# matthewT53/JPEG-Encoder-and-Decoder

Hardware: AMD Instinct MI355X
Metric: Mpixels/sec RGB→quantised-coeff, 4K 4:4:4 q=90; % HBM roofline (higher is better)
Workload: dtype f32; 1 GPU; 8 x 3840x2160 RGB frames per GPU, 4:4:4, q=90, block-row stripes; global_batch_frames=8, width=3840, height=2160, quality=90, parallelism=stripes1, collectives=none, kernel_timing=HIP events around the K launches on their stream, launch=eager, input_sets=2

## Files before the change

jpeg-encoder-and-decoder_amd/csrc/jpgx_internal.h:

```cpp
#ifndef JPGX_INTERNAL_H
#define JPGX_INTERNAL_H

#include <stddef.h>
#include <stdint.h>

#include "../../include/jpgx.h"

#define JX_WG 256

struct jx_udiv {
    uint32_t m, s1, s2;
};
static inline struct jx_udiv jx_udiv_make(uint32_t d)
{
    unsigned l = 0;
    while (l < 32 && (1ull << l) < (unsigned long long)d) l++;
    struct jx_udiv r;
    r.m = (uint32_t)(((1ull << 32) * ((1ull << l) - d)) / d + 1);
    r.s1 = l ? 1u : 0u;
    r.s2 = l ? l - 1u : 0u;
    return r;
}

struct jx_geom {
    const uint8_t *rgb;
    int16_t *out;
    long long in_pitch;
    long long in_fstride;
    long long out_fstride;
    int bpr;
    int nb;
    int nframes;
    int row0;
    uint32_t under[6];
    struct jx_udiv dnb, dbpr;
    uint32_t mpr, nmcu;
    struct jx_udiv dmpr, dnmcu;
};

struct jx_qtab {
    float w[3][8][8];
    int16_t q[2][64];
};

struct jx_limtab {
    float lim[3][8][8];
};

#define JX_MAXQ 97

#ifndef JX_MX_PARTS
#define JX_MX_PARTS 2
#endif
#ifndef JX_MX_LOEXP
#define JX_MX_LOEXP 0
#endif
struct jx_mxtab {
    float w[24][8];
    float lsq[24][8];
    int16_t q[2][64];
    double r[2][64];
};

struct jx_xform_args {
    struct jx_geom g;
    int quality;
    int force_exact;
    int luma_only;
    int sub;
};


#ifdef __cplusplus
extern "C" {
#endif
int jx_plan_tables(int quality, float w[3][64], float lim[3][64], int16_t q[2][64]);
int jx_plan_tables_mode(int quality, int sub, float w[3][64], float lim[3][64], int16_t q[2][64]);
void jx_under_dwords(const uint8_t under[3][8], uint32_t out[6]);
long long jx_selftest_pk(long long nblocks, unsigned long long seed);
int jx_mx_parts(void);
int jx_mx_loexp(void);
int jx_plan_tables_mx(int quality, float w[24][8], float lim[24][8], int16_t q[2][64]);
int jx_plan_tables_mx422(int quality, float w[24][8], float lim[24][8], int16_t q[2][64]);
int jx_plan_tables_mx420(int quality, float w[24][8], float lim[24][8], int16_t q[2][64]);
int jx_mx_operands(uint16_t ops[3 * JX_MX_PARTS][64][8]);
int jx_mx422_operands(uint16_t ops[JX_MX_PARTS][4][64][8]);
int jx_mx420_operands(uint16_t ops[JX_MX_PARTS][5][64][8]);
long long jx_selftest_mx(long long nblocks, unsigned long long seed, int quality,
                         long long *flagged, double *ratio);
long long jx_selftest_mx422(long long nblocks, unsigned long long seed, int quality,
                            long long *flagged, double *ratio);
long long jx_selftest_mx420(long long nblocks, unsigned long long seed, int quality,
                            long long *flagged, double *ratio);
int jx_launch_mx(const struct jx_xform_args *xa, int sr, void *stream, void *ev_start, void *ev_stop);
long long jx_mx_image(int sr, int force, int quality, void *dst, long long cap);
int jx_launch_alt(const struct jx_xform_args *xa, int sr, size_t nbc, void *stream, void *ev_start, void *ev_stop);
#define JX_JFIF_HDR_MAX 768
void jx_jfif_build_codes(const uint8_t bits[16], const uint8_t *vals, uint32_t cl[256]);
void jx_jfif_codes(uint32_t cl[4][256]);
size_t jx_jfif_header(int width, int height, int quality, int sample_ratio, unsigned ri,
                      uint8_t *out, size_t cap);
#define JX_JFIF_DHT_STD 432
size_t jx_jfif_header_tabs(int width, int height, int quality, int sample_ratio, unsigned ri,
                           const uint8_t bits[4][16], const uint8_t vals[4][256], uint8_t *out,
                           size_t cap, size_t *dht_at);
int jx_jfif_optimal(const uint64_t counts[256], uint8_t bits[16], uint8_t vals[256]);
#ifdef __cplusplus
}
#endif

#endif
```

jpeg-encoder-and-decoder_amd/csrc/jpgx_mx.hip:

```cpp
#include <hip/hip_ext.h>
#include <hip/hip_runtime.h>
#include <math.h>
#include <stdint.h>
#include <string.h>

#include <algorithm>
#include <memory>
#include <mutex>
#include <type_traits>
#include <vector>

#include "jpgx_internal.h"
#include "jx_consts.h"
#include "jx_hip.h"
#include "xform_math.h"

#pragma clang fp contract(off)

namespace {

typedef _Float16 mx_h8 __attribute__((ext_vector_type(8)));
typedef _Float16 mx_h2 __attribute__((ext_vector_type(2)));
typedef float mx_f4 __attribute__((ext_vector_type(4)));
typedef uint32_t mx_u4 __attribute__((ext_vector_type(4)));
// ... 339 lines not shown
        if (__popc(b1) == 1 && one(sl, (unsigned)__builtin_ctz(b1))) bits = 0;
    }
}

__device__ __forceinline__ bool mx_put_one(const void *stage, unsigned off, bool ok, int val)
{
    if (!__builtin_amdgcn_readfirstlane((int)ok)) return false;
    if (mx_lane() == 0) *(__attribute__((address_space(3))) int16_t *)(mx_lds((void *)stage) + off) = (int16_t)val;
    return true;
}

__device__ __forceinline__ unsigned mx_col_block(unsigned k, unsigned sl)
{
    const unsigned gg = sl >> 4, jj = sl & 15u;
    return k == 0 ? gg : (k == 1 ? 4u + gg : (jj < 8 ? gg : 4u + gg));
}

template <class Lds, class XT>
__device__ __forceinline__ void mx_exact_inline(Lds &L, const uint8_t *slot, uint32_t bits,
                                                const XT &xt)
{
    const unsigned lane = mx_lane();
    mx_wave_sync();
    mx_exact_single(bits, [&](unsigned sl, unsigned bt) __attribute__((always_inline)) {
        const unsigned k = bt >> 3, v = bt & 7u;
        const unsigned jj = sl & 15u, u = jj & 7u, ch = k < 2 ? (jj >> 3) : 2u;
        const unsigned jb = mx_col_block(k, sl);
        int val;
        const bool ok = mx_exact_one(MxSmp1{mx_lds((void *)slot) + 24u * jb, 192u}, ch, u, v, xt, val);
        return mx_put_one(L.stage, mxs_coef(mx_pos(ch, jb), xt.scan(u, v)), ok, val);
    });
    for (;;) {
        const uint64_t act = __ballot(bits != 0);
        if (!act) break;
        const int rk = mx_rank(act);
        if (bits != 0 && rk < 8) {
            const unsigned b = (unsigned)__builtin_ctz(bits);
            bits &= bits - 1u;
            L.task[rk] = (uint16_t)(lane << 8 | b);
        }
        mx_wave_sync();
        const int nt = std::min((int)__popcll(act), 8);
        const unsigned i = lane >> 3, x = lane & 7u;
        const bool live = (int)i < nt;
        const unsigned code = L.task[live ? i : 0u];
        const unsigned sl = code >> 8, k = (code >> 3) & 3u, v = code & 7u;
        const unsigned jj = sl & 15u, u = jj & 7u, ch = k < 2 ? (jj >> 3) : 2u;
        const unsigned jb = mx_col_block(k, sl);
        const int val = mx_exact_coef<true>(MxSmp1{mx_lds((void *)slot) + 24u * jb, 192u}, ch, u, v, x, xt);
        if (live && x == 7)
            *(__attribute__((address_space(3))) int16_t *)(mx_lds(L.stage) + mxs_coef(mx_pos(ch, jb), xt.scan(u, v))) =
                (int16_t)val;
        mx_wave_sync();
    }
}

__device__ __forceinline__ void mx_unpack8(const mx_f4 &a, const mx_f4 &b, float (&o)[8])
{
    o[0] = a.x, o[4] = a.y, o[2] = a.z, o[6] = a.w;
    o[1] = b.x, o[3] = b.y, o[5] = b.z, o[7] = b.w;
}

__device__ __forceinline__ uint32_t mx_flags(const float (&F)[8], const float (&W)[8], const float (&Lq)[8])
{
    uint32_t m = 0;
#pragma unroll
    for (int k = 0; k < 8; k++) {
        const float tm = __builtin_fmaf(F[k], W[k], kMagic);
        const float rr = tm - kMagic;
        const float d = __builtin_fmaf(F[k], W[k], -rr);
        const float e = __builtin_fmaf(d, d, -Lq[k]);
        m |= (e >= 0.0f ? 1u : 0u) << k;
    }
    return m;
}

static_assert(JX_MX_LOEXP == 0, "the kernels take R = acc_h + acc_l");
__device__ __forceinline__ void mx_combine(mx_f4 hl, mx_f4 ll, mx_f4 hh, mx_f4 lh, float (&R)[8])
{
    R[0] = ll.x + hl.x, R[1] = ll.y + hl.y, R[2] = ll.z + hl.z, R[3] = ll.w + hl.w;
    R[4] = lh.x + hh.x, R[5] = lh.y + hh.y, R[6] = lh.z + hh.z, R[7] = lh.w + hh.w;
}

struct MxW {
    mx_f4 w01, w23;
};
__device__ __forceinline__ MxW mx_w(const MxTab &tb, unsigned t0, unsigned j)
{
    return MxW{tb.wl[t0][0][j], tb.wl[t0][1][j]};
}
__device__ __forceinline__ MxW mx_l(const MxTab &tb, unsigned t0, unsigned j)
{
    return MxW{tb.wl[t0 + 1][0][j], tb.wl[t0 + 1][1][j]};
}
struct MxsTab {
    mx_f4 yc[2][2][16];
    mx_f4 cr[2][2][8];
};
__device__ __forceinline__ MxW mx_w(const MxsTab &tb, unsigned t0, unsigned j)
{
    return t0 == 0 ? MxW{tb.yc[0][0][j], tb.yc[0][1][j]} : MxW{tb.cr[0][0][j & 7u], tb.cr[0][1][j & 7u]};
}
__device__ __forceinline__ MxW mx_l(const MxsTab &tb, unsigned t0, unsigned j)
{
    return t0 == 0 ? MxW{tb.yc[1][0][j], tb.yc[1][1][j]} : MxW{tb.cr[1][0][j & 7u], tb.cr[1][1][j & 7u]};
}
__host__ __device__ __forceinline__ float mx_limc(const MxTab &tb, unsigned t, unsigned j)
{
    const mx_f4 a = tb.wl[t][0][j], b = tb.wl[t][1][j];
    const float mn = fminf(fminf(fminf(a.x, a.y), fminf(a.z, a.w)), fminf(fminf(b.x, b.y), fminf(b.z, b.w)));
    if (!(mn >= 0.0f)) return -1.0f;
    return (float)sqrt((double)mn) * (1.0f - 0x1p-20f);
}

__device__ __forceinline__ void mx_fence(const mx_f4 &r)
{
    const uint32_t v = __builtin_amdgcn_readfirstlane(__float_as_uint(r.w));
    asm volatile("" ::"s"(v) : "memory");
}

template <int N>
__device__ __forceinline__ void mx_fence_all(const mx_f4 (&r)[N])
{
    uint32_t v = 0;
#pragma unroll
    for (int i = 0; i < N; i++) v += __float_as_uint(r[i].w);
    asm volatile("" ::"v"(v) : "memory");
}

__device__ __forceinline__ void mx_keep(const mx_f4 (&x)[4])
{
    asm volatile("" ::"v"(x[0]), "v"(x[1]), "v"(x[2]), "v"(x[3]));
}
template <class T>
__device__ __forceinline__ int mx_keep1(const T &x)
{
    asm volatile("" ::"v"(x));
    return 0;
}
template <class... T>
__device__ __forceinline__ void mx_keep_ops(const T &...x)
{
    const int k[] = {mx_keep1(x)...};
    (void)k;
}

template <unsigned OFF, class TB>
__device__ __forceinline__ void mx_column_r(const float (&R)[8], const MxW &t, float limc, const TB &tb,
                                             unsigned t0, unsigned j, const uint32_t (&za)[8], uint32_t &fl, int kc,
                                             const mx_f4 *fence = nullptr)
{
    float F[8], W[8];
    jx_fdct8<FOps>(R, F);
    mx_unpack8(t.w01, t.w23, W);
    typedef __attribute__((address_space(3))) uint16_t l16;
    float em = 0.0f;
#pragma unroll
    for (int p = 0; p < 4; p++) {
        const int k0 = jx_pk_k(p, 0), k1 = jx_pk_k(p, 1);
        const float t0v = __builtin_fmaf(F[k0], W[k0], kMagic), t1v = __builtin_fmaf(F[k1], W[k1], kMagic);
        *(l16 *)(uintptr_t)(za[k0] + OFF) = (uint16_t)__float_as_uint(t0v);
        *(l16 *)(uintptr_t)(za[k1] + OFF) = (uint16_t)__float_as_uint(t1v);
        const float d0 = __builtin_fmaf(F[k0], W[k0], -(t0v - kMagic));
        const float d1 = __builtin_fmaf(F[k1], W[k1], -(t1v - kMagic));
        em = __builtin_fmaxf(__builtin_fmaxf(em, __builtin_fabsf(d0)), __builtin_fabsf(d1));
    }
    if (__builtin_expect(__ballot(em >= limc) != 0, 0)) {
        if (fence) mx_fence(*fence);
        const MxW lw = mx_l(tb, t0, j);
        float Lq[8];
        mx_unpack8(lw.w01, lw.w23, Lq);
        fl |= mx_flags(F, W, Lq) << (8 * kc);
    }
}

struct MxNoKeep {
    __device__ void operator()() const {}
};
template <unsigned OFF, bool LAZY = false, class TB, class KF = MxNoKeep>
__device__ __forceinline__ void mx_column_t(const mx_f4 (&acc)[4], const MxW &t, float limc, const TB &tb,
                                             unsigned t0, unsigned j, const uint32_t (&za)[8], uint32_t &fl, int kc,
                                             const mx_f4 *fence = nullptr, const KF &keep = KF{})
{
    float R[8];
    mx_combine(acc[0], acc[1], acc[2], acc[3], R);
    if (LAZY) {
        __builtin_amdgcn_sched_barrier(0);
        if (fence) mx_fence(*fence);
        keep();
        mx_column_r<OFF>(R, mx_w(tb, t0, j), limc, tb, t0, j, za, fl, kc, nullptr);
    } else {
        keep();
        mx_column_r<OFF>(R, t, limc, tb, t0, j, za, fl, kc, fence);
    }
}

constexpr unsigned kMxsC = 3;
constexpr unsigned kMxsWPG = 4;
struct alignas(16) MxsLds {
    uint8_t ring[kMxsC][kSlot];
    uint8_t stage[24 * kBSs];
    uint16_t task[8];
};
static_assert(sizeof(MxsLds) % 16 == 0, "16-byte aligned LDS regions");
__device__ mx_u4 g_mxs_B[3 * JX_MX_PARTS][64];
struct alignas(16) MxsImg {
    MxsTab tab;
    float limc[2][16];
    uint8_t scan_t[8][8];
    MxExTab ex;
};
constexpr unsigned kMxsPieces = sizeof(MxsImg) / 16;
static_assert(sizeof(MxsImg) % 16 == 0 && kMxsPieces <= 768, "three 16-byte pieces per thread");
static_assert(sizeof(MxsLds) * kMxsWPG + sizeof(MxsImg) <= 40 * 1024, "4 workgroups of 4 waves per CU");
__device__ MxsImg g_mxs_img[2][JX_MAXQ + 1];

template <unsigned N>
__device__ __forceinline__ void mx_wait_vm()
{
    static_assert(N < 64, "vmcnt is 6 bits");
    __builtin_amdgcn_s_waitcnt((int)((N & 15u) | ((N >> 4) << 14) | 0xF70u));
}

template <int SIZE>
__device__ __forceinline__ void mxs_dma(const void *g, void *lds)
{
    static_assert(SIZE == 16 || SIZE == 4, "dwordx4 or dword pieces");
    if constexpr (SIZE == 16)
        __builtin_amdgcn_global_load_lds((mx_gp)g, (mx_lp)lds, 16, 0, 0);
    else
        __builtin_amdgcn_global_load_lds((mx_gp)g, (mx_lp)lds, 4, 0, 0);
}

struct MxsCur {
    unsigned b, c;
    bool simple;
    const uint8_t *src;
    int16_t *dst;
    int16_t *cdst;
};

__device__ __forceinline__ void mxs_simple(MxsCur &P, const MxG &g)
{
    P.simple = P.c + 8u < g.bpr && P.b + 8u <= g.total && g.lin_store;
}

__device__ __forceinline__ void mxs_at(MxsCur &P, const MxG &g, unsigned b)
{
    P.b = b;
    P.simple = false;
    if (b >= g.total) return;
    MxCur X;
    mx_seek(X, g, b);
    P.c = X.c;
    P.src = X.src;
    P.dst = X.dst;
    P.cdst = g.out + (long long)X.f * g.ofstride + 64ll * (g.nb + X.bi / 2u);
    mxs_simple(P, g);
}

__device__ __forceinline__ void mxs_next(MxsCur &P, const MxG &g)
{
    if (!P.simple) {
        mxs_at(P, g, P.b + 8u);
        return;
    }
    P.b += 8u;
    P.c += 8u;
    P.src += 192;
    P.dst += 512;
    P.cdst += 256;
    mxs_simple(P, g);
}

__device__ __forceinline__ void mxs_issue(const MxsCur &P, const MxG &g, uint8_t *slot, uint32_t off0,
                                          uint32_t off1, unsigned lane)
{
    if (P.simple) {
        mxs_dma<16>(P.src + off0, slot);
        if (lane < 32) mxs_dma<16>(P.src + off1, slot + 1024u);
    } else {
        mxs_dma<4>(g.rgb, slot);
        mxs_dma<4>(g.rgb, slot);
    }
}

__global__ __launch_bounds__(64 * kMxsWPG, kWPE) void k_mxs(const jx_xform_args a)
{
    __shared__ __attribute__((aligned(16))) MxsLds s_lds[kMxsWPG];
    __shared__ __attribute__((aligned(16))) MxsImg s_img;
    MxG g;
    g.rgb = a.g.rgb;
    g.out = a.g.out;
    g.pitch = a.g.in_pitch;
    g.fstride = a.g.in_fstride;
    g.ofstride = a.g.out_fstride;
    g.bpr = (unsigned)a.g.bpr;
    g.nb = (unsigned)a.g.nb;
    g.total = (unsigned)a.g.nb * (unsigned)a.g.nframes;
    g.row0 = a.g.row0;
    g.quality = a.quality;
    g.force = a.force_exact;
    g.lin_store = (unsigned long long)g.nb * 256ull + 1024ull < (1ull << 31);
#pragma unroll
    for (int k = 0; k < 6; k++) g.u[k] = a.g.under[k];
    g.dnb = a.g.dnb;
    g.dbpr = a.g.dbpr;

    const unsigned lane = threadIdx.x & 63u;
    const unsigned wave = __builtin_amdgcn_readfirstlane(threadIdx.x >> 6);
    MxsLds &L = s_lds[wave];
    mx_u4 B[kParts][3];
#pragma unroll
    for (int p = 0; p < kParts; p++)
#pragma unroll
        for (int w = 0; w < 3; w++) B[p][w] = g_mxs_B[3 * p + w][lane];
    {
        const uint8_t *img = (const uint8_t *)&g_mxs_img[g.force ? 1 : 0][g.quality];
#pragma unroll
        for (unsigned i = 0; i < (kMxsPieces + 64u * kMxsWPG - 1u) / (64u * kMxsWPG); i++) {
            const unsigned piece = 64u * kMxsWPG * i + threadIdx.x;
            if (64u * kMxsWPG * i + 64u * wave < kMxsPieces && piece < kMxsPieces)
                mxs_dma<16>(img + 16u * piece, (uint8_t *)&s_img + 16u * (64u * kMxsWPG * i + 64u * wave));
        }
    }
    const unsigned wv = blockIdx.x * kMxsWPG + wave;
    const uint32_t off0 = (uint32_t)((lane / 12u) * (unsigned)g.pitch + 16u * (lane % 12u));
    const uint32_t off1 = (uint32_t)(((64u + lane) / 12u) * (unsigned)g.pitch + 16u * ((64u + lane) % 12u));
    MxsCur iss;
    mxs_at(iss, g, 8u * kMxsC * wv);
    MxsCur cmp = iss;
#pragma unroll
    for (unsigned k = 0; k < kMxsC; k++) {
        mxs_issue(iss, g, L.ring[k], off0, off1, lane);
        mxs_next(iss, g);
    }

    const unsigned m = lane & 15u, q = lane >> 4;
    const uint32_t aoff = 192u * (m & 3u) + 24u * (m >> 2) + 8u * (q < 3 ? q : 2u);
    const uint32_t s0 = q < 3 ? kSelLo : kSelOne;
    const uint32_t s1 = q < 3 ? kSelHi : kSelZero;
    const uint32_t s2 = q < 3 ? kSelLo : kSelZero;
    const uint32_t so0 = lane * 16u, so1 = so0 + g.nb * 128u, so2 = so1 + g.nb * 128u;
    const uint32_t ro = mx_ro(lane);
    const uint32_t rr = (ro ^ (lane & 32u)) + 1024u + ((lane & 32u) << 5);
    const uint32_t rcb = (ro ^ 32u) + 1536u;
    const unsigned gq = lane >> 4, j = lane & 15u, u = j & 7u;
    const MxExLds xt{s_img.ex, s_img.scan_t};

    mx_wait_vm<2u * kMxsC>();
    __builtin_amdgcn_s_barrier();
    mx_wave_sync();
    if (cmp.b >= g.total) {
        mx_wait_vm<0>();
        return;
    }
    uint32_t za[8];
    {
        const unsigned s = mx_pos(j >> 3, gq);
        const uint32_t base = (uint32_t)(uintptr_t)mx_lds(L.stage) + kBSs * s, hs = mxs_h(s);
        const mx_u2 sc = *(const mx_u2 *)&s_img.scan_t[u][0];
#pragma unroll
        for (int v = 0; v < 8; v++) {
            const uint32_t z = (v < 4 ? sc.x : sc.y) >> (8 * (v & 3)) & 0xffu;
            za[v] = base + 16u * ((z >> 3) ^ hs) + 2u * (z & 7u);
        }
    }
    const float limc0 = s_img.limc[0][j], limc2 = s_img.limc[1][j];
    const MxsTab &tb = s_img.tab;

    const auto body = [&](const MxsCur &S, uint8_t *sp) __attribute__((always_inline)) {
        if (!S.simple) {
            MxCur P;
            mx_seek(P, g, S.b);
            mx_issue(g, P, S.b, false, off0, off1, sp);
        }
        mx_wave_sync();
        const mx_u2 d00 = *(const mx_u2 *)(sp + aoff);
        const mx_u2 d01 = *(const mx_u2 *)(sp + aoff + 768u);
        const mx_u2 d10 = *(const mx_u2 *)(sp + aoff + 96u);
        const mx_u2 d11 = *(const mx_u2 *)(sp + aoff + 864u);
        const MxW w0 = mx_w(tb, 0, j);
        const mx_h8 A00 = mx_aop(d00, s0, s1, s2), A01 = mx_aop(d01, s0, s1, s2);
        const mx_h8 A10 = mx_aop(d10, s0, s1, s2), A11 = mx_aop(d11, s0, s1, s2);
        __builtin_amdgcn_sched_barrier(0);
        const mx_f4 z = {};
        uint32_t fl = 0;
        mx_f4 acc[3][4];
        const auto mma_set = [&](mx_f4(&o)[4], const mx_h8 &Alo, const mx_h8 &Ahi) __attribute__((always_inline)) {
            o[0] = mx_mma(Alo, B[0][0], z);
            o[2] = mx_mma(Ahi, B[0][0], z);
            o[1] = mx_mma(Alo, B[1][0], z);
            o[3] = mx_mma(Ahi, B[1][0], z);
        };
        mma_set(acc[0], A00, A01);
        __builtin_amdgcn_sched_barrier(0);
        mma_set(acc[1], A10, A11);
        __builtin_amdgcn_sched_barrier(0);
        mx_column_t<0>(acc[0], w0, limc0, tb, 0, j, za, fl, 0);
        __builtin_amdgcn_sched_barrier(0);
        mx_f4 cr[2][4];
        cr[0][0] = mx_mma(A00, B[0][1], z);
        __builtin_amdgcn_sched_barrier(0);
        cr[0][2] = mx_mma(A01, B[0][1], z);
        __builtin_amdgcn_sched_barrier(0);
        cr[0][1] = mx_mma(A00, B[1][1], z);
        __builtin_amdgcn_sched_barrier(0);
        cr[0][3] = mx_mma(A01, B[1][1], z);
        __builtin_amdgcn_sched_barrier(0);
        cr[1][0] = mx_mma(A10, B[0][2], z);
        __builtin_amdgcn_sched_barrier(0);
        cr[1][2] = mx_mma(A11, B[0][2], z);
        __builtin_amdgcn_sched_barrier(0);
        cr[1][1] = mx_mma(A10, B[1][2], z);
        __builtin_amdgcn_sched_barrier(0);
        cr[1][3] = mx_mma(A11, B[1][2], z);
        __builtin_amdgcn_sched_barrier(0);
        mx_column_t<4 * kBSs>(acc[1], w0, limc0, tb, 0, j, za, fl, 1, &cr[1][3]);
        __builtin_amdgcn_sched_barrier(0);
        const uint8_t *const ob = (const uint8_t *)S.dst;
        const auto clamp = [&](uint32_t &f) __attribute__((always_inline)) {
            if (S.b + 8u > g.total) {
                const unsigned nvalid = g.total - S.b;
#pragma unroll
                for (int kk = 0; kk < 3; kk++)
                    if (mx_col_block((unsigned)kk, lane) >= nvalid) f &= ~(0xffu << (8 * kk));
            }
        };
        const auto store = [&](int c) __attribute__((always_inline)) {
            const unsigned l = mx_lane();
            const unsigned bl = S.b + (l >> 3), b = bl < g.total ? bl : g.total - 1u;
            const unsigned f = b / g.nb, bi = b - f * g.nb;
            const mx_u4 val = *(const mx_u4 *)(L.stage + mxs_piece(mx_pos((unsigned)c, l >> 3), l & 7u));
            if (bl < g.total)
                __builtin_nontemporal_store(
                    val, (mx_u4 *)(g.out + (long long)f * g.ofstride + ((long long)c * g.nb + bi) * 64 + (l & 7u) * 8));
        };
        const bool early = S.simple && __ballot((fl & 0xffffu) != 0) == 0;
        if (early) {
            mx_fence(cr[1][3]);
            mx_wave_sync();
            const mx_u4 v0 = *(const mx_u4 *)(L.stage + ro);
            const mx_u4 v1 = *(const mx_u4 *)(L.stage + rcb);
            __builtin_nontemporal_store(v0, (mx_u4 *)(ob + so0));
            __builtin_nontemporal_store(v1, (mx_u4 *)(ob + so1));
        }
        __builtin_amdgcn_sched_barrier(0);
#pragma unroll
        for (int i = 0; i < 4; i++)
            acc[2][i] = mx_f4{cr[0][i].x + cr[1][i].x, cr[0][i].y + cr[1][i].y, cr[0][i].z + cr[1][i].z,
                              cr[0][i].w + cr[1][i].w};
        mx_column_t<8 * kBSs, true>(acc[2], w0, limc2, tb, 2, j, za, fl, 2);
        mx_wave_sync();
        if (__builtin_expect(__ballot(fl != 0) != 0, 0)) {
            clamp(fl);
            mx_exact_inline(L, sp, fl, xt);
        }
        if (early) {
            const mx_u4 v2 = *(const mx_u4 *)(L.stage + rr);
            __builtin_nontemporal_store(v2, (mx_u4 *)(ob + so2));
        } else if (S.simple) {
            const mx_u4 v0 = *(const mx_u4 *)(L.stage + ro);
            const mx_u4 v1 = *(const mx_u4 *)(L.stage + rcb);
            const mx_u4 v2 = *(const mx_u4 *)(L.stage + rr);
            __builtin_nontemporal_store(v0, (mx_u4 *)(ob + so0));
            __builtin_nontemporal_store(v1, (mx_u4 *)(ob + so1));
            __builtin_nontemporal_store(v2, (mx_u4 *)(ob + so2));
        } else {
#pragma unroll
            for (int c = 0; c < 3; c++) store(c);
        }
        mx_wave_sync();
    };

    const auto step = [&](auto kc) __attribute__((always_inline)) {
        constexpr unsigned k = decltype(kc)::value;
        if (cmp.b >= g.total) {
            mx_wait_vm<0>();
            return;
        }
        mx_wait_vm<2 * (kMxsC - 1 - k) + 3 * k>();
        body(cmp, L.ring[k]);
        mxs_next(cmp, g);
    };
    step(std::integral_constant<unsigned, 0>{});
    step(std::integral_constant<unsigned, 1>{});
    step(std::integral_constant<unsigned, 2>{});
}

constexpr unsigned kSt422C = 8 * kBS2;

__device__ __forceinline__ unsigned mx422_yblock(unsigned sl)
{
    return (sl & 15u) < 8 ? (sl >> 4) : 4u + (sl >> 4);
}

template <class Lds>
__device__ __forceinline__ MxSmp2 mx422_smp(Lds &L, const uint8_t *sp, uint32_t qmask, unsigned cb)
{
    const bool q = (qmask >> cb) & 1u;
    const lds_u8 *pl = mx_lds((void *)sp) + 48u * cb;
    return MxSmp2{pl, q ? mx_lds(L.qtrue[cb]) : pl + 24u, 192u, q ? 24u : 192u};
}

template <class Lds, class XT>
__device__ __forceinline__ void mx422_exact_inline(Lds &L, const uint8_t *sp, uint32_t qmask,
                                                   uint32_t bits, const XT &xt)
{
    const unsigned lane = mx_lane();
    mx_wave_sync();
    mx_exact_single(bits, [&](unsigned sl, unsigned bt) __attribute__((always_inline)) {
        const unsigned k = bt >> 3, v = bt & 7u, jj = sl & 15u, u = jj & 7u;
        const unsigned slot = mx422_yblock(sl);
        int val;
        bool ok;
        if (k == 0)
            ok = mx_exact_one(MxSmp1{mx_lds((void *)sp) + 24u * slot, 192u}, 0u, u, v, xt, val);
        else
            ok = mx_exact_one(mx422_smp(L, sp, qmask, sl >> 4), 1u + (jj >> 3), u, v, xt, val);
        return mx_put_one(L.stage, mx2_coef(slot + (k ? 8u : 0u), xt.scan(u, v)), ok, val);
    });
    for (;;) {
        const uint64_t act = __ballot(bits != 0);
        if (!act) break;
        const int rk = mx_rank(act);
        if (bits != 0 && rk < 8) {
            const unsigned b = (unsigned)__builtin_ctz(bits);
            bits &= bits - 1u;
            L.task[rk] = (uint16_t)(lane << 8 | b);
        }
        mx_wave_sync();
        const int nt = std::min((int)__popcll(act), 8);
        const unsigned i = lane >> 3, x = lane & 7u;
        const bool live = (int)i < nt;
        const unsigned code = L.task[live ? i : 0u];
// ... 790 lines not shown
            for (int v = 0; v < 8; v++) {
                const double K = (u == 0 ? qa0 : 0.25) * (v == 0 ? JX_ALPHA0 : 1.0);
                t.r[c][u * 8 + v] = K / (double)t.q[c][u * 8 + v];
            }
}

typedef int (*mx_plan_fn)(int, float[24][8], float[24][8], int16_t[2][64]);
constexpr mx_plan_fn kMxPlan[3] = {jx_plan_tables_mx, jx_plan_tables_mx422, jx_plan_tables_mx420};

int mx_plan_tabs(std::vector<jx_mxtab> &tab, int mode, int qlo, int qhi)
{
    tab.assign(2 * (JX_MAXQ + 1), jx_mxtab{});
    for (int q = qlo; q <= qhi; q++) {
        float w[24][8], lim[24][8];
        int16_t qq[2][64];
        const int rc = kMxPlan[mode](q, w, lim, qq);
        if (rc) return rc;
        for (int f = 0; f < 2; f++) {
            jx_mxtab &t = tab[f * (JX_MAXQ + 1) + q];
            memcpy(t.q, qq, sizeof qq);
            mx_fill_recip(t);
            for (int n = 0; n < 24; n++)
                for (int v = 0; v < 8; v++) {
                    t.w[n][v] = w[n][v] * kRScale;
                    t.lsq[n][v] = f ? -1.0f : mx_lsq(lim[n][v]);
                }
        }
    }
    return JPGX_OK;
}

template <class Col>
void mx_layout_tab(MxTab &o, const jx_mxtab &t, Col ncol)
{
    for (unsigned tt = 0; tt < 4; tt++)
        for (unsigned jp = 0; jp < 16; jp++) {
            const unsigned n = ncol(tt, jp);
            float x[8];
            for (int pp = 0; pp < 4; pp++)
                for (int h = 0; h < 2; h++) {
                    const int v = jx_pk_k(pp, h);
                    x[2 * pp + h] = (tt & 1u) ? t.lsq[n][v] : t.w[n][v];
                }
            o.wl[tt][0][jp] = mx_f4{x[0], x[1], x[2], x[3]};
            o.wl[tt][1][jp] = mx_f4{x[4], x[5], x[6], x[7]};
        }
}

void mx_scan_t(uint8_t (&st)[8][8])
{
    static const int scan[8][8] = JX_SCAN_ORDER_INIT;
    for (int uu = 0; uu < 8; uu++)
        for (int v = 0; v < 8; v++) st[uu][v] = (uint8_t)scan[v][uu];
}

void mx_ex_tab(MxExTab &x, const jx_mxtab &t)
{
    static const double cosx[8][8] = JX_COS_INIT;
    memcpy(x.cosx_, cosx, sizeof cosx);
    memcpy(x.q_, t.q, sizeof t.q);
    memcpy(x.r_, t.r, sizeof t.r);
}

typedef uint16_t mx_tile[64][8];

struct MxsK {
    typedef MxsImg Img;
    static constexpr const char *name = "k_mxs";
    static constexpr int mode = 0;
    static constexpr unsigned tiles = 3, pair = 1, wpg = kMxsWPG, unit = 1, per_wave = 8 * kMxsC;
    static auto kernel() { return k_mxs; }
    static auto &symbol() { return g_mxs_img; }
    static unsigned ncol(unsigned tt, unsigned jp) { return tt < 2 ? jp : 16u + (jp & 7u); }
    static int operands(mx_tile *ops) { return jx_mx_operands(ops); }
    static void land(Img &I, const MxTab &full, const mx_tile *)
    {
        for (unsigned jp = 0; jp < 16; jp++)
            for (int tt = 0; tt < 2; tt++)
                for (int h = 0; h < 2; h++) {
                    I.tab.yc[tt][h][jp] = full.wl[tt][h][jp];
                    if (jp < 8) I.tab.cr[tt][h][jp] = full.wl[2 + tt][h][jp];
                }
    }
    static hipError_t upload_operands(const mx_tile *ops)
    {
        return hipMemcpyToSymbol(HIP_SYMBOL(g_mxs_B), ops, sizeof(mx_tile) * tiles * JX_MX_PARTS);
    }
};

template <class ImgT, int SUB>
struct MxsSubK {
    typedef ImgT Img;
    static constexpr int mode = SUB;
    static constexpr unsigned tiles = 3 + SUB, pair = 0;
    static unsigned ncol(unsigned tt, unsigned jp) { return tt < 2 ? (jp & 7u) : 8u + jp; }
    static void land(Img &I, const MxTab &full, const mx_tile *ops)
    {
        I.tab = full;
        for (unsigned p = 0; p < JX_MX_PARTS; p++)
            for (unsigned l = 0; l < 64; l++) {
                memcpy(&I.B[(tiles - 1) * p][l], ops[tiles * p + ((l & 15u) < 8 ? 0 : 1)][l], 16);
                for (unsigned w = 2; w < tiles; w++) memcpy(&I.B[(tiles - 1) * p + w - 1][l], ops[tiles * p + w][l], 16);
            }
    }
    static hipError_t upload_operands(const mx_tile *) { return hipSuccess; }
};

struct Mxs422K : MxsSubK<MxsImg422, 1> {
    static constexpr const char *name = "k_mxs422";
    static constexpr unsigned wpg = kMxs422WPG, unit = 1, per_wave = 8 * kMxs422C;
    static auto kernel() { return k_mxs422; }
    static auto &symbol() { return g_mxs422_img; }
    static int operands(mx_tile *ops) { return jx_mx422_operands((uint16_t(*)[4][64][8])ops); }
};

struct Mxs420K : MxsSubK<MxsImg420, 2> {
    static constexpr const char *name = "k_mxs420";
    static constexpr unsigned wpg = kMxs420WPG, unit = 4, per_wave = 8;
    static auto kernel() { return k_mxs420; }
    static auto &symbol() { return g_mxs420_img; }
    static int operands(mx_tile *ops) { return jx_mx420_operands((uint16_t(*)[5][64][8])ops); }
};

template <class F>
auto mx_for_kernel(int sr, F f)
{
    return sr == 1 ? f(Mxs422K{}) : sr == 2 ? f(Mxs420K{}) : f(MxsK{});
}

template <class K>
int mx_build_images(std::vector<typename K::Img> &img, std::vector<uint16_t> &opsv, int qlo, int qhi)
{
    typedef typename K::Img Img;
    std::vector<jx_mxtab> tab;
    int rc = mx_plan_tabs(tab, K::mode, qlo, qhi);
    opsv.assign(sizeof(mx_tile) / sizeof(uint16_t) * K::tiles * JX_MX_PARTS, 0);
    mx_tile *ops = (mx_tile *)opsv.data();
    if (!rc) rc = K::operands(ops);
    if (rc) return rc;
    for (unsigned p = 0; p < JX_MX_PARTS; p++)
        for (unsigned l = 0; l < 64; l++)
            for (int e = 0; e < 8; e++)
                if (ops[K::tiles * p + K::pair + ((l & 15u) < 8 ? 1 : 0)][l][e]) return JPGX_EARG;
    img.resize(2 * (JX_MAXQ + 1));
    memset(img.data(), 0, img.size() * sizeof(Img));
    for (int f = 0; f < 2; f++)
        for (int q = qlo; q <= qhi; q++) {
            Img &I = img[f * (JX_MAXQ + 1) + q];
            const jx_mxtab &t = tab[f * (JX_MAXQ + 1) + q];
            MxTab full;
            mx_layout_tab(full, t, K::ncol);
            for (unsigned jp = 0; jp < 16; jp++) {
                I.limc[0][jp] = mx_limc(full, 1, jp);
                I.limc[1][jp] = mx_limc(full, 3, jp);
            }
            K::land(I, full, ops);
            mx_scan_t(I.scan_t);
            mx_ex_tab(I.ex, t);
        }
    return JPGX_OK;
}

template <class K>
int mx_tables_for_current_device()
{
    static std::once_flag once[JX_MAX_DEV];
    static int rcs[JX_MAX_DEV];
    int dev = 0;
    if (hipGetDevice(&dev) != hipSuccess || dev < 0 || dev >= JX_MAX_DEV) return JPGX_ENODEV;
// ... 58 lines not shown
```

jpeg-encoder-and-decoder_amd/csrc/jpgx_plan.cpp:

```cpp
#include <math.h>
#include <string.h>

#include <algorithm>
#include <memory>

#include "jpgx_internal.h"
#include "jx_consts.h"
#include "xform_math.h"

static const int kLum[8][8] = JX_Q_LUM_INIT;
static const int kChr[8][8] = JX_Q_CHR_INIT;

namespace {

struct Bnd {
    double lo, hi, E;
};

struct BoundOps {
    typedef Bnd T;
    static double mag(const Bnd &a) { return std::max(fabs(a.lo), fabs(a.hi)); }
    static Bnd round_(double lo, double hi, double err)
    {
        const double u = 0x1p-24;
// ... 346 lines not shown
static long double mx_exact(int mode, int k, int n)
{
    if (n >= mx_ncol(mode) || k > mx_nk(mode)) return 0;
    const long double pi = 3.141592653589793238462643383279502884L;
    const int u = n % 8;
    if (mode == 0) {
        const int c = n / 8;
        if (k < 24) {
            const int x = k / 3, p = k % 3;
            return (long double)kMxA[c][p] * cosl((2 * x + 1) * u * pi / 16);
        }
        return u == 0 && c == 0 ? -1024.0L : 0;
    }
    if (k == mx_nk(mode)) return 0;
    const int c = 1 + n / 8, kk = k % 48, x = kk / 3, p = kk % 3;
    return (mode == 1 ? 0.5L : 0.25L) * (long double)kMxA[c][p] * cosl((2 * (x / 2) + 1) * u * pi / 16);
}

constexpr int kMxBExp = 15, kMxBiasExp = -9;
static long double mx_enc(long double v, bool bias, uint16_t *bits)
{
    const int e = bias ? kMxBiasExp : kMxBExp;
    return ldexpl(f16_round(ldexpl(v, e), bits), -e);
}

struct MxSplit {
    int mode, nk, ncol;
    long double h[97][24], l[97][24], m[97][24];
    uint16_t bh[97][24], bl[97][24], bm[97][24];
    uint16_t bits(int part, int k, int n) const
    {
        return k > nk ? 0 : (part == 0 ? bh[k][n] : (part == 1 ? bl[k][n] : bm[k][n]));
    }
};
typedef std::unique_ptr<MxSplit> MxSplitPtr;

static int mx_split(int mode, MxSplit &S)
{
    memset(&S, 0, sizeof S);
    S.mode = mode;
    S.nk = mx_nk(mode);
    S.ncol = mx_ncol(mode);
    for (int k = 0; k <= S.nk; k++)
        for (int n = 0; n < S.ncol; n++) {
            const long double B = mx_exact(mode, k, n);
            const bool bias = k == S.nk;
            const long double hv = mx_enc(bias ? B : rintl(ldexpl(B, 11)) / 2048.0L, bias, &S.bh[k][n]);
            if (ldexpl(hv, 11) != rintl(ldexpl(hv, 11))) return JPGX_EARG;
            S.h[k][n] = hv;
            const long double ls = mx_enc(ldexpl(B - hv, JX_MX_LOEXP), bias, &S.bl[k][n]);
            S.l[k][n] = ldexpl(ls, -JX_MX_LOEXP);
            if (JX_MX_PARTS == 3) {
                const long double ms = mx_enc(ldexpl(B - hv, JX_MX_LOEXP) - ls, bias, &S.bm[k][n]);
                S.m[k][n] = ldexpl(ms, -JX_MX_LOEXP);
            }
        }
    for (int n = 0; n < S.ncol; n++) {
        long double sh = fabsl(S.h[S.nk][n]);
        for (int k = 0; k < S.nk; k++) sh += 255.0L * fabsl(S.h[k][n]);
        if (sh >= 8192.0L) return JPGX_EARG;
    }
    return JPGX_OK;
}

extern "C" int jx_mx_parts(void) { return JX_MX_PARTS; }
extern "C" int jx_mx_loexp(void) { return JX_MX_LOEXP; }

extern "C" int jx_mx_operands(uint16_t ops[3 * JX_MX_PARTS][64][8])
{
    MxSplitPtr S(new MxSplit);
    const int rc = mx_split(0, *S);
    if (rc) return rc;
    for (int part = 0; part < JX_MX_PARTS; part++)
        for (int which = 0; which < 3; which++)
            for (int l = 0; l < 64; l++)
                for (int e = 0; e < 8; e++) {
                    const int k = 8 * (l >> 4) + e, j = l & 15;
                    int n = -1;
                    if (which == 0) n = j;
                    else if (which == 1 && j < 8) n = 16 + j;
                    else if (which == 2 && j >= 8) n = 16 + j - 8;
                    ops[3 * part + which][l][e] = n >= 0 ? S->bits(part, k, n) : 0;
                }
    return JPGX_OK;
}

static int mxc_operands(int mode, uint16_t *ops)
{
    MxSplitPtr Y(new MxSplit), C(new MxSplit);
    int rc = mx_split(0, *Y);
    if (!rc) rc = mx_split(mode, *C);
    if (rc) return rc;
    const int nwhich = 2 + mx_products(mode);
    for (int part = 0; part < JX_MX_PARTS; part++)
        for (int which = 0; which < nwhich; which++)
            for (int l = 0; l < 64; l++)
                for (int e = 0; e < 8; e++) {
                    const int j = l & 15, k = 8 * (l >> 4) + e;
                    uint16_t v = 0;
                    if (which >= 2) v = C->bits(part, 32 * (which - 2) + k, j);
                    else if (which == 0 ? j < 8 : j >= 8) v = Y->bits(part, k, j & 7);
                    ops[((part * nwhich + which) * 64 + l) * 8 + e] = v;
                }
    return JPGX_OK;
}

extern "C" int jx_mx422_operands(uint16_t ops[JX_MX_PARTS][4][64][8]) { return mxc_operands(1, &ops[0][0][0][0]); }
extern "C" int jx_mx420_operands(uint16_t ops[JX_MX_PARTS][5][64][8]) { return mxc_operands(2, &ops[0][0][0][0]); }

static Bnd mx_row_bound(const MxSplit &S, int n)
{
    const int nk = S.nk;
    long double loh = S.h[nk][n], hih = S.h[nk][n];
    long double lol = S.l[nk][n] + S.m[nk][n], hil = lol;
    long double sl = fabsl(S.l[nk][n]) + fabsl(S.m[nk][n]);
    long double rep = fabsl(mx_exact(S.mode, nk, n) - S.h[nk][n] - S.l[nk][n] - S.m[nk][n]);
    for (int k = 0; k < nk; k++) {
        const long double bh = S.h[k][n], bo = S.l[k][n] + S.m[k][n];
        loh += std::min(0.0L, 255.0L * bh);
        hih += std::max(0.0L, 255.0L * bh);
        lol += std::min(0.0L, 255.0L * bo);
        hil += std::max(0.0L, 255.0L * bo);
        sl += 255.0L * (fabsl(S.l[k][n]) + fabsl(S.m[k][n]));
        rep += 255.0L * fabsl(mx_exact(S.mode, k, n) - S.h[k][n] - S.l[k][n] - S.m[k][n]);
    }
    const double nadd = 2.0 * ((32.0 * mx_products(S.mode) + 1.0) * (JX_MX_PARTS - 1));
    const double el = (double)(nadd * sl * 0x1p-23L + rep);
    return BoundOps::add(Bnd{(double)loh, (double)hih, 0.0},
                         Bnd{(double)lol - el, (double)hil + el, el});
}

static int mx_plan_tables(int mode, int quality, float w[24][8], float lim[24][8], int16_t q[2][64])
{
    int qs[2][8][8];
    int rc = plan_divisors(quality, qs, q);
    if (rc) return rc;
    MxSplitPtr Y(new MxSplit), C;
    rc = mx_split(0, *Y);
    if (!rc && mode) {
        C.reset(new MxSplit);
        rc = mx_split(mode, *C);
    }
    if (rc) return rc;
    const long double a0 = 1.0L / sqrtl(2.0L);
    for (int n = 0; n < 24; n++) {
        const int c = n / 8, u = n % 8, t = c == 0 ? 0 : 1;
        const Bnd R = mode == 0 || c == 0 ? mx_row_bound(*Y, n) : mx_row_bound(*C, n - 8);
        Bnd col[8], out[8];
        for (int y = 0; y < 8; y++) col[y] = R;
        jx_fdct8<BoundOps>(col, out);
        for (int v = 0; v < 8; v++) {
            const long double au = u == 0 ? a0 : 1.0L, av = v == 0 ? a0 : 1.0L;
            const long double ws = 0.25L * au * av * dct_kfactor(v) / (long double)qs[t][u][v];
            plan_band(ws, out[v], &w[n][v], &lim[n][v]);
        }
    }
    return JPGX_OK;
}

extern "C" int jx_plan_tables_mx(int quality, float w[24][8], float lim[24][8], int16_t q[2][64])
{
    return mx_plan_tables(0, quality, w, lim, q);
}

extern "C" int jx_plan_tables_mx422(int quality, float w[24][8], float lim[24][8], int16_t q[2][64])
{
// ... 117 lines not shown
```

Measured before the change: 611,900 Mpixels/s.

## Pack chroma hi/lo operand parts into one tile and combine via DPP

After: 625,400 Mpixels/s, median of 6. 2.2% higher.

```diff
diff --git a/jpeg-encoder-and-decoder_amd/csrc/jpgx_internal.h b/jpeg-encoder-and-decoder_amd/csrc/jpgx_internal.h
--- a/jpeg-encoder-and-decoder_amd/csrc/jpgx_internal.h
+++ b/jpeg-encoder-and-decoder_amd/csrc/jpgx_internal.h
@@ -84,6 +84,7 @@
 int jx_plan_tables_mx422(int quality, float w[24][8], float lim[24][8], int16_t q[2][64]);
 int jx_plan_tables_mx420(int quality, float w[24][8], float lim[24][8], int16_t q[2][64]);
 int jx_mx_operands(uint16_t ops[3 * JX_MX_PARTS][64][8]);
+int jx_mxs_device_operands(uint16_t out[3][64][8]);
 int jx_mx422_operands(uint16_t ops[JX_MX_PARTS][4][64][8]);
 int jx_mx420_operands(uint16_t ops[JX_MX_PARTS][5][64][8]);
 long long jx_selftest_mx(long long nblocks, unsigned long long seed, int quality,
diff --git a/jpeg-encoder-and-decoder_amd/csrc/jpgx_mx.hip b/jpeg-encoder-and-decoder_amd/csrc/jpgx_mx.hip
--- a/jpeg-encoder-and-decoder_amd/csrc/jpgx_mx.hip
+++ b/jpeg-encoder-and-decoder_amd/csrc/jpgx_mx.hip
@@ -445,6 +445,20 @@
     R[4] = lh.x + hh.x, R[5] = lh.y + hh.y, R[6] = lh.z + hh.z, R[7] = lh.w + hh.w;
 }
 
+__device__ __forceinline__ float mxs_cr_row(float x, float y)
+{
+    float r = y + __builtin_bit_cast(float, __builtin_amdgcn_update_dpp(0, __builtin_bit_cast(int, y), 0x128, 0xf, 0xf, true));
+    asm("v_add_f32_dpp %0, %1, %1 row_ror:8 row_mask:0xf bank_mask:0x3" : "+v"(r) : "v"(x));
+    return r;
+}
+__device__ __forceinline__ void mxs_cr_rows(const mx_f4 (&cx)[2][2], float (&R)[8])
+{
+    R[0] = mxs_cr_row(cx[0][0].x, cx[1][0].x), R[1] = mxs_cr_row(cx[0][0].y, cx[1][0].y);
+    R[2] = mxs_cr_row(cx[0][0].z, cx[1][0].z), R[3] = mxs_cr_row(cx[0][0].w, cx[1][0].w);
+    R[4] = mxs_cr_row(cx[0][1].x, cx[1][1].x), R[5] = mxs_cr_row(cx[0][1].y, cx[1][1].y);
+    R[6] = mxs_cr_row(cx[0][1].z, cx[1][1].z), R[7] = mxs_cr_row(cx[0][1].w, cx[1][1].w);
+}
+
 struct MxW {
     mx_f4 w01, w23;
 };
@@ -566,7 +580,7 @@
     uint16_t task[8];
 };
 static_assert(sizeof(MxsLds) % 16 == 0, "16-byte aligned LDS regions");
-__device__ mx_u4 g_mxs_B[3 * JX_MX_PARTS][64];
+__device__ mx_u4 g_mxs_B[3][64];
 struct alignas(16) MxsImg {
     MxsTab tab;
     float limc[2][16];
@@ -673,11 +687,9 @@
     const unsigned lane = threadIdx.x & 63u;
     const unsigned wave = __builtin_amdgcn_readfirstlane(threadIdx.x >> 6);
     MxsLds &L = s_lds[wave];
-    mx_u4 B[kParts][3];
-#pragma unroll
-    for (int p = 0; p < kParts; p++)
-#pragma unroll
-        for (int w = 0; w < 3; w++) B[p][w] = g_mxs_B[3 * p + w][lane];
+    mx_u4 B[3];
+#pragma unroll
+    for (int w = 0; w < 3; w++) B[w] = g_mxs_B[w][lane];
     {
         const uint8_t *img = (const uint8_t *)&g_mxs_img[g.force ? 1 : 0][g.quality];
 #pragma unroll
@@ -749,12 +761,12 @@
         __builtin_amdgcn_sched_barrier(0);
         const mx_f4 z = {};
         uint32_t fl = 0;
-        mx_f4 acc[3][4];
+        mx_f4 acc[2][4];
         const auto mma_set = [&](mx_f4(&o)[4], const mx_h8 &Alo, const mx_h8 &Ahi) __attribute__((always_inline)) {
-            o[0] = mx_mma(Alo, B[0][0], z);
-            o[2] = mx_mma(Ahi, B[0][0], z);
-            o[1] = mx_mma(Alo, B[1][0], z);
-            o[3] = mx_mma(Ahi, B[1][0], z);
+            o[0] = mx_mma(Alo, B[0], z);
+            o[2] = mx_mma(Ahi, B[0], z);
+            o[1] = mx_mma(Alo, B[1], z);
+            o[3] = mx_mma(Ahi, B[1], z);
         };
         mma_set(acc[0], A00, A01);
         __builtin_amdgcn_sched_barrier(0);
@@ -762,24 +774,16 @@
         __builtin_amdgcn_sched_barrier(0);
         mx_column_t<0>(acc[0], w0, limc0, tb, 0, j, za, fl, 0);
         __builtin_amdgcn_sched_barrier(0);
-        mx_f4 cr[2][4];
-        cr[0][0] = mx_mma(A00, B[0][1], z);
-        __builtin_amdgcn_sched_barrier(0);
-        cr[0][2] = mx_mma(A01, B[0][1], z);
-        __builtin_amdgcn_sched_barrier(0);
-        cr[0][1] = mx_mma(A00, B[1][1], z);
-        __builtin_amdgcn_sched_barrier(0);
-        cr[0][3] = mx_mma(A01, B[1][1], z);
-        __builtin_amdgcn_sched_barrier(0);
-        cr[1][0] = mx_mma(A10, B[0][2], z);
-        __builtin_amdgcn_sched_barrier(0);
-        cr[1][2] = mx_mma(A11, B[0][2], z);
-        __builtin_amdgcn_sched_barrier(0);
-        cr[1][1] = mx_mma(A10, B[1][2], z);
-        __builtin_amdgcn_sched_barrier(0);
-        cr[1][3] = mx_mma(A11, B[1][2], z);
-        __builtin_amdgcn_sched_barrier(0);
-        mx_column_t<4 * kBSs>(acc[1], w0, limc0, tb, 0, j, za, fl, 1, &cr[1][3]);
+        mx_f4 cx[2][2];
+        cx[0][0] = mx_mma(A00, B[2], z);
+        __builtin_amdgcn_sched_barrier(0);
+        cx[0][1] = mx_mma(A01, B[2], z);
+        __builtin_amdgcn_sched_barrier(0);
+        cx[1][0] = mx_mma(A10, B[2], z);
+        __builtin_amdgcn_sched_barrier(0);
+        cx[1][1] = mx_mma(A11, B[2], z);
+        __builtin_amdgcn_sched_barrier(0);
+        mx_column_t<4 * kBSs>(acc[1], w0, limc0, tb, 0, j, za, fl, 1, &cx[1][1]);
         __builtin_amdgcn_sched_barrier(0);
         const uint8_t *const ob = (const uint8_t *)S.dst;
         const auto clamp = [&](uint32_t &f) __attribute__((always_inline)) {
@@ -801,7 +805,7 @@
         };
         const bool early = S.simple && __ballot((fl & 0xffffu) != 0) == 0;
         if (early) {
-            mx_fence(cr[1][3]);
+            mx_fence(cx[1][1]);
             mx_wave_sync();
             const mx_u4 v0 = *(const mx_u4 *)(L.stage + ro);
             const mx_u4 v1 = *(const mx_u4 *)(L.stage + rcb);
@@ -809,11 +813,12 @@
             __builtin_nontemporal_store(v1, (mx_u4 *)(ob + so1));
         }
         __builtin_amdgcn_sched_barrier(0);
-#pragma unroll
-        for (int i = 0; i < 4; i++)
-            acc[2][i] = mx_f4{cr[0][i].x + cr[1][i].x, cr[0][i].y + cr[1][i].y, cr[0][i].z + cr[1][i].z,
-                              cr[0][i].w + cr[1][i].w};
-        mx_column_t<8 * kBSs, true>(acc[2], w0, limc2, tb, 2, j, za, fl, 2);
+        {
+            float R[8];
+            mxs_cr_rows(cx, R);
+            __builtin_amdgcn_sched_barrier(0);
+            mx_column_r<8 * kBSs>(R, mx_w(tb, 2, j), limc2, tb, 2, j, za, fl, 2);
+        }
         mx_wave_sync();
         if (__builtin_expect(__ballot(fl != 0) != 0, 0)) {
             clamp(fl);
@@ -1770,9 +1775,12 @@
                     if (jp < 8) I.tab.cr[tt][h][jp] = full.wl[2 + tt][h][jp];
                 }
     }
-    static hipError_t upload_operands(const mx_tile *ops)
+    static hipError_t upload_operands(const mx_tile *)
     {
-        return hipMemcpyToSymbol(HIP_SYMBOL(g_mxs_B), ops, sizeof(mx_tile) * tiles * JX_MX_PARTS);
+        std::vector<uint16_t> dev(sizeof(mx_tile) / sizeof(uint16_t) * 3);
+        static_assert(sizeof(g_mxs_B) == 3 * sizeof(mx_tile), "the three device tiles");
+        if (jx_mxs_device_operands((mx_tile *)dev.data())) return hipErrorInvalidValue;
+        return hipMemcpyToSymbol(HIP_SYMBOL(g_mxs_B), dev.data(), sizeof(g_mxs_B));
     }
 };
 
diff --git a/jpeg-encoder-and-decoder_amd/csrc/jpgx_plan.cpp b/jpeg-encoder-and-decoder_amd/csrc/jpgx_plan.cpp
--- a/jpeg-encoder-and-decoder_amd/csrc/jpgx_plan.cpp
+++ b/jpeg-encoder-and-decoder_amd/csrc/jpgx_plan.cpp
@@ -452,6 +452,21 @@
                     else if (which == 2 && j >= 8) n = 16 + j - 8;
                     ops[3 * part + which][l][e] = n >= 0 ? S->bits(part, k, n) : 0;
                 }
+    return JPGX_OK;
+}
+
+static_assert(JX_MX_PARTS == 2, "k_mxs's Cr tile holds one hi and one lo part");
+extern "C" int jx_mxs_device_operands(uint16_t out[3][64][8])
+{
+    std::unique_ptr<uint16_t[][64][8]> ops(new uint16_t[3 * JX_MX_PARTS][64][8]);
+    const int rc = jx_mx_operands(ops.get());
+    if (rc) return rc;
+    for (int l = 0; l < 64; l++)
+        for (int e = 0; e < 8; e++) {
+            out[0][l][e] = ops[0][l][e];
+            out[1][l][e] = ops[3][l][e];
+            out[2][l][e] = (l & 15) < 8 ? ops[3 * 0 + 1][l][e] : ops[3 * 1 + 2][l][e];
+        }
     return JPGX_OK;
 }
 
```
